# guptakhil/show-tell

Measured on AMD Instinct MI355X. Metric: training images/sec (ResNet101+GRU, emb=512, bs=128) at 1/2/4/8 MI355X, higher is better.
Workload: dtype bf16; 1 GPU; BASELINE configs[1]: ResNet-101 (train-mode BN, frozen) + 5-layer GRU decoder, E=H=512, V=10000, fwd+bwd+SGD step, synthetic COCO-shaped batch; batch_per_gpu=128, global_batch=128, image=3x224x224, parallelism=dp1

## Files before the change

### include/showtell_hip.h

```cpp
#ifndef SHOWTELL_HIP_H
#define SHOWTELL_HIP_H

#include <stddef.h>
#include <stdint.h>

#ifdef __cplusplus
extern "C" {
#endif

#define ST_F32 0
#define ST_BF16 1

#define ST_CELL_GRU 0
#define ST_CELL_LSTM 1

const char* st_last_error(void);
int st_version(void);

typedef struct {
  const void* x;
  const void* w;
  void* y;
  const float* bias;
  const float* scale;
// ... 51 lines not shown
#endif
typedef struct {
  const void* raw2; const void* w3_frag; const void* identity; void* x_out; const void* w1_frag; void* y;
  float* stats; int stats_replicas;
  const float* bn2_stats; const float* bn2_gamma; const float* bn2_beta; int bn2_replicas;
  const float* bn3_stats; const float* bn3_gamma; const float* bn3_beta; int bn3_replicas;
  const float* id_stats; const float* id_gamma; const float* id_beta; int id_replicas;
  float count; float eps;
  long rows; int C1, C2, N;
} st_conv_b2b_desc;
int st_conv_b2b_supported(int C1, int C2, int N);
int st_conv_b2b(const st_conv_b2b_desc* d, void* stream);
typedef struct {
  const void* x2; const void* w3_frag; const void* identity; void* x_out; const void* w1_frag; void* y;
  float* stats; int stats_replicas;
  const float* bn2_stats; const float* bn2_gamma; const float* bn2_beta; int bn2_replicas;
  const float* bn3_stats; const float* bn3_gamma; const float* bn3_beta; int bn3_replicas;
  float count; float eps;
  const float* scale3; const float* shift3; const float* scale1; const float* shift1; int relu1;
  long rows; int C1, C2, N;
  const float* id_stats; const float* id_gamma; const float* id_beta; int id_replicas;
} st_conv_c3c1_desc;
int st_conv_c3c1_supported(int C1, int C2, int N);
int st_conv_c3c1(const st_conv_c3c1_desc* d, void* stream);
int st_conv1x1_astat_supported(int C, int N);
int st_conv1x1_astat(const st_conv1x1_wreg_desc* d, void* stream);

int st_pack_conv_weight_frag(const float* w, void* out, int Cout, int Cin, int KH, int KW, int ntw, void* stream);

int st_tune(int reserved, int kc, int w8);
int st_prof_enable(int on);
int st_debug_stamps(unsigned long long* buf);
int st_prof_collect(double* ms, double* flops, long* launches);

typedef struct {
  const void* x; void* y; const void* res;
  const float* stats;  const float* gamma; const float* beta;
  const float* running_mean; const float* running_var;
  const float* res_stats; const float* res_gamma; const float* res_beta;
  const float* res_running_mean; const float* res_running_var;
  int res_bn;
  int dtype; long rows; int C; float count; float eps; int relu;
  int stats_replicas, res_stats_replicas;
} st_bn_act_desc;

int st_bn_act(const st_bn_act_desc* d, void* stream);

int st_bn_update_running(const float* stats, float* running_mean, float* running_var,
                         int C, float count, float momentum, void* stream);

int st_nchw_to_nhwc(const float* x, void* y, int dtype, int B, int C, int H, int W, int Cpad, void* stream);
int st_nchw_to_s2d16(const float* x, void* y, int dtype, int B, int H, int W, void* stream);
int st_stem_weight_s2d(const void* w, void* out, int dtype, int Cpad, void* stream);
int st_nhwc_to_ncp_f32(const void* x, float* y, int dtype, int B, int HW, int C, void* stream);
int st_maxpool3x3s2(const void* x, void* y, int dtype, int B, int H, int W, int C, void* stream);
int st_maxpool3x3s2_bn(const void* x, void* y, int dtype, int B, int H, int W, int C,
                       const float* stats, const float* gamma, const float* beta,
                       const float* running_mean, const float* running_var, float count, float eps, void* stream);
typedef struct {
  const void* x_s2d; const void* w_frag; void* y;
  float* stats; int stats_replicas;
  const float* gamma;
  const float* scale; const float* shift;
  int B, H, W;
} st_stem_conv_pool_desc;
int st_stem_conv_pool(const st_stem_conv_pool_desc* d, void* stream);
// ... 174 lines not shown
```

### show-tell_amd/_lib.py

```python
import ctypes as C
import os

_HERE = os.path.dirname(os.path.abspath(__file__))
LIB_PATH = os.path.join(_HERE, "lib", "libshowtell_hip.so")

ST_F32, ST_BF16 = 0, 1
ST_CELL_GRU, ST_CELL_LSTM = 0, 1

c_p, c_i, c_f, c_l = C.c_void_p, C.c_int, C.c_float, C.c_long


class ConvDesc(C.Structure):
    _fields_ = [("x", c_p), ("w", c_p), ("y", c_p), ("bias", c_p), ("scale", c_p), ("shift", c_p),
                ("residual", c_p), ("stats", c_p), ("dtype", c_i), ("out_dtype", c_i),
                ("B", c_i), ("Hin", c_i), ("Win", c_i), ("Cin", c_i), ("Ho", c_i), ("Wo", c_i), ("N", c_i),
                ("KH", c_i), ("KW", c_i), ("stride", c_i), ("pad", c_i),
                ("ldx", c_i), ("ldw", c_i), ("ldy", c_i), ("relu", c_i), ("accumulate", c_i), ("Cin_logical", c_i), ("k_order", c_i), ("stats_replicas", c_i),
                ("in_stats", c_p), ("in_gamma", c_p), ("in_beta", c_p), ("in_count", c_f), ("in_eps", c_f), ("split_k", c_i)]


class Conv3x3ImgDesc(C.Structure):
    _fields_ = [("x", c_p), ("w_frag", c_p), ("y", c_p), ("stats", c_p), ("stats_replicas", c_i), ("scale", c_p), ("shift", c_p),
                ("relu", c_i), ("in_stats", c_p), ("in_gamma", c_p), ("in_beta", c_p), ("in_count", c_f), ("in_eps", c_f),
                ("B", c_i), ("H", c_i), ("W", c_i), ("C", c_i), ("N", c_i), ("in_stats_replicas", c_i)]
# ... 75 lines not shown
                ("rows_b", c_p), ("rows_t", c_p), ("prev_row", c_p), ("caption", c_p)]


class ImageBatchDesc(C.Structure):
    _fields_ = [("src", c_p), ("src_bytes", C.c_int64), ("offset", c_p), ("height", c_p), ("width", c_p), ("flip", c_p), ("batch", c_i),
                ("max_height", c_i), ("max_width", c_i), ("out_h", c_i), ("out_w", c_i), ("lut", c_p), ("tmp", c_p),
                ("out", c_p), ("out_u8", c_p)]


_SIGS = {
    "st_version": ([], c_i),
    "st_image_transform": ([C.POINTER(ImageBatchDesc), c_p], c_i),
    "st_conv": ([C.POINTER(ConvDesc), c_p], c_i),
    "st_conv_batch": ([C.POINTER(ConvDesc), c_i, c_p], c_i),
    "st_conv3x3_img_supported": ([c_i, c_i, c_i, c_i], c_i),
    "st_conv3x3_img": ([C.POINTER(Conv3x3ImgDesc), c_p], c_i),
    "st_conv3x3_s2_supported": ([c_i, c_i], c_i),
    "st_conv3x3_s2": ([C.POINTER(Conv3x3ImgDesc), c_p], c_i),
    "st_conv1x1_wreg_supported": ([c_i, c_i], c_i),
    "st_conv1x1_wreg": ([C.POINTER(Conv1x1WregDesc), c_p], c_i),
    "st_conv1x1_kfuse": ([C.POINTER(Conv1x1KfuseDesc), c_p], c_i),
    "st_conv1x1_kfuse_supported": ([c_i, c_i], c_i),
    "st_conv1x1_kfuse8": ([C.POINTER(Conv1x1KfuseDesc), c_p], c_i),
    "st_conv_b2b": ([C.POINTER(ConvB2bDesc), c_p], c_i),
    "st_conv_b2b_supported": ([c_i, c_i, c_i], c_i),
    "st_conv1x1_astat_supported": ([c_i, c_i], c_i),
    "st_conv1x1_astat": ([C.POINTER(Conv1x1WregDesc), c_p], c_i),
    "st_conv1x1_kstream_supported": ([c_i, c_i], c_i),
    "st_conv1x1_kstream": ([C.POINTER(Conv1x1WregDesc), c_p], c_i),
    "st_pack_conv_weight_frag": ([c_p, c_p, c_i, c_i, c_i, c_i, c_i, c_p], c_i),
    "st_tune": ([c_i, c_i, c_i], c_i),
    "st_prof_enable": ([c_i], c_i),
    "st_debug_stamps": ([c_p], c_i),
    "st_prof_collect": ([C.POINTER(C.c_double), C.POINTER(C.c_double), C.POINTER(c_l)], c_i),
    "st_bn_act": ([C.POINTER(BnActDesc), c_p], c_i),
    "st_bn_update_running": ([c_p, c_p, c_p, c_i, c_f, c_f, c_p], c_i),
    "st_nchw_to_nhwc": ([c_p, c_p, c_i, c_i, c_i, c_i, c_i, c_i, c_p], c_i),
    "st_nchw_to_s2d16": ([c_p, c_p, c_i, c_i, c_i, c_i, c_p], c_i),
    "st_stem_weight_s2d": ([c_p, c_p, c_i, c_i, c_p], c_i),
    "st_stem_weight_frag": ([c_p, c_p, c_p], c_i),
    "st_stem_weight_frag_packed": ([c_p, c_i, c_p, c_p], c_i),
    "st_stem_conv_pool": ([C.POINTER(StemConvPoolDesc), c_p], c_i),
    "st_nhwc_to_ncp_f32": ([c_p, c_p, c_i, c_i, c_i, c_i, c_p], c_i),
    "st_maxpool3x3s2": ([c_p, c_p, c_i, c_i, c_i, c_i, c_i, c_p], c_i),
    "st_maxpool3x3s2_bn": ([c_p, c_p, c_i, c_i, c_i, c_i, c_i, c_p, c_p, c_p, c_p, c_p, c_f, c_f, c_p], c_i),
    "st_global_avgpool": ([c_p, c_p, c_i, c_i, c_i, c_i, c_i, c_p], c_i),
    "st_cast": ([c_p, c_p, c_i, c_i, c_l, c_p], c_i),
    "st_transpose": ([c_p, c_p, c_i, c_i, c_i, c_i, c_i, c_p], c_i),
    "st_transpose_colsum": ([c_p, c_p, c_p, c_i, c_i, c_i, c_i, c_i, c_p], c_i),
    "st_transpose_batch": ([c_p, c_p, c_p, c_i, c_i, c_i, c_i, c_i, c_i, c_p, c_p, c_p], c_i),
    "st_pack_conv_weight": ([c_p, c_p, c_i, c_i, c_i, c_i, c_i, c_i, c_i, c_p], c_i),
    "st_cast2d": ([c_p, c_p, c_i, c_i, c_i, c_i, c_i, c_i, c_p], c_i),
    "st_rnn_vocab_ld": ([c_i], c_i),
    "st_rnn_workspace_bytes": ([C.POINTER(RnnParams), C.POINTER(PackedSeq)], C.c_size_t),
    "st_rnn_forward": ([C.POINTER(RnnParams), C.POINTER(PackedSeq), c_p, c_p, c_p, C.c_size_t, c_p, c_i, c_i, c_p, c_i, c_p], c_i),
    "st_rnn_fused_loss_supported": ([C.POINTER(RnnParams)], c_i),
    "st_rnn_fused_loss_bytes": ([C.POINTER(RnnParams), C.POINTER(PackedSeq)], C.c_size_t),
    "st_rnn_fused_loss": ([C.POINTER(RnnParams), C.POINTER(PackedSeq), c_p, C.c_size_t, c_p, c_p, C.c_size_t, c_p, c_p], c_i),
    "st_rnn_fused_dlogits": ([C.POINTER(RnnParams), C.POINTER(PackedSeq), c_p, C.c_size_t, c_p, c_p, c_p, c_p, c_i, c_p], c_i),
    "st_rnn_backward": ([C.POINTER(RnnParams), C.POINTER(RnnGrads), C.POINTER(PackedSeq), c_p, c_p, c_i, c_p, c_p, C.c_size_t,
                         c_p, c_p, c_p], c_i),
    "st_rnn_greedy_workspace_bytes": ([C.POINTER(RnnParams), c_i], C.c_size_t),
    "st_rnn_greedy": ([C.POINTER(RnnParams), c_p, c_i, c_i, c_p, C.c_size_t, c_p, c_p, c_p], c_i),
    "st_rnn_greedy_last_route": ([], c_i),
    "st_rnn_step": ([C.POINTER(RnnParams), c_p, c_i, c_p, c_p, c_p, c_p, c_p, c_i, c_p], c_i),
    "st_embedding_rows": ([c_p, c_p, c_p, c_i, c_i, c_i, c_i, c_i, c_p], c_i),
# ... 80 lines not shown
```

### show-tell_amd/csrc/conv_img.hip

```cpp
#include "common.h"
#include "prof.h"
#include <stdlib.h>
#include <stdio.h>

namespace {

struct ImgArgs {
  const bf16_t* x; const bf16_t* w; bf16_t* y;
  float* stats; int srep;
  const float* scale; const float* shift; int relu;
  const float* in_stats; const float* in_gamma; const float* in_beta; float in_count, in_eps; int in_srep;
  int B, H, W, N, Wp, R, bands, nbn;
  unsigned long long* stamps;
};

template <int CTRL> __device__ __forceinline__ float dpp_rot_(float v) {
  return __int_as_float(__builtin_amdgcn_update_dpp(0, __float_as_int(v), CTRL, 0xf, 0xf, true));
}
__device__ __forceinline__ float row16_sum_(float v) {
  v += dpp_rot_<0x128>(v); v += dpp_rot_<0x124>(v); v += dpp_rot_<0x122>(v); v += dpp_rot_<0x121>(v);
  return v;
}
__device__ __forceinline__ f32x4 mfma_bf16(const u32x4& a, const u32x4& b, const f32x4& c) {
  return __builtin_amdgcn_mfma_f32_16x16x32_bf16(*reinterpret_cast<const bf16x8*>(&a), *reinterpret_cast<const bf16x8*>(&b), c, 0, 0, 0);
}

template <int NC, int BNLOC>
__device__ __forceinline__ void block_stats_flush(const float (&es)[NC], const float (&ess)[NC], bool writer, int local, char* smem,
                                                  float* sdst, int chan0, int N, int tid) {
  float* sred = reinterpret_cast<float*>(smem);
  __syncthreads();
  if (writer) {
#pragma unroll
    for (int c = 0; c < NC; ++c) { sred[local + c] = es[c]; sred[BNLOC + local + c] = ess[c]; }
  }
  __syncthreads();
  for (int t = tid; t < 2 * BNLOC; t += 256) atomicAdd(sdst + (t < BNLOC ? chan0 + t : N + chan0 + t - BNLOC), sred[t]);
}

__device__ __forceinline__ void bn_relu_chunk(u32x4& v, const float* sc, const float* sh);

template <int C, int TM, int NTW, int HALVES, bool AFFINE, int MS = 1>
__device__ __forceinline__ void conv3x3_img_body(const ImgArgs& a) {
  constexpr int TMW = TM / MS;
  static_assert(TM % MS == 0 && (MS == 1 || MS == 2) && (MS == 1 || HALVES == 1), "position split");
  constexpr int PIX = 2 * C + 32;
  constexpr int CS = C / 32;
  constexpr int CSH = CS / HALVES;
  constexpr int KS = 9 * CS;
  constexpr int CH8 = C / 8;
  constexpr int PSTEP = 256 / CH8;
  constexpr bool ALLW = KS * NTW * 4 <= 96;
  extern __shared__ __attribute__((aligned(16))) char smem[];

  const int tid = threadIdx.x, lane = tid & 63;
  const int wid = __builtin_amdgcn_readfirstlane(tid >> 6);
  int lid;
  {
    const int nblk = gridDim.x, id = blockIdx.x, xcd = id & 7, q = nblk >> 3, r = nblk & 7;
    lid = (xcd < r ? xcd * (q + 1) : r * (q + 1) + (xcd - r) * q) + (id >> 3);
  }
  const int nb = lid % a.nbn;
  const int bi = lid / a.nbn;
  const int band = bi % a.bands, img = bi / a.bands;
  const int r0 = band * a.R;
  const int rows = a.H - r0 < a.R ? a.H - r0 : a.R;
  const int Wp = a.Wp;

#define IMG_STAMP(i) do { if (a.stamps && lane == 0) a.stamps[((size_t)blockIdx.x * 4 + wid) * 8 + (i)] = __builtin_amdgcn_s_memtime(); } while (0)
  IMG_STAMP(0);
  constexpr int NSH = C > 256 ? C / 256 : 1;
  StatHead shd[NSH];
  if (a.in_stats) {
#pragma unroll
    for (int k = 0; k < NSH; ++k) { const int c = (tid + 256 * k) % C; stat_head_issue(shd[k], a.in_stats, a.in_srep, C, c, a.in_gamma, a.in_beta); }
  }
  const int r16 = lane & 15, q4 = lane >> 4;
  const int wn = MS == 1 ? wid : (wid & 1), wm = MS == 1 ? 0 : (wid >> 1);
  const int T0 = (nb * (4 / MS) + wn) * NTW;
  const u32x4* wl = reinterpret_cast<const u32x4*>(a.w) + lane;
  constexpr int WQ = ALLW ? KS : CS;
  u32x4 wq[WQ][NTW];
#pragma unroll
  for (int s = 0; s < WQ; ++s)
#pragma unroll
    for (int j = 0; j < NTW; ++j) wq[s][j] = wl[((size_t)(T0 + j) * KS + s) * 64];

  constexpr int CHH = CH8 / 2, U2 = TM >= 14 ? 19 : TM + 3;
  u32x4 v1[HALVES == 2 ? U2 : 1]; bool ok1[HALVES == 2 ? U2 : 1];
  float sc1[8], sh1[8];
  const int cch2 = tid % CHH, pp2 = tid / CHH;
  const bool xf_ = a.in_stats != nullptr;
  if constexpr (HALVES == 2) {
    const int total = 16 * TM + 2 * Wp + 2;
    float* coef = reinterpret_cast<float*>(smem + (size_t)total * PIX);
    const bf16_t* ximg = a.x + (size_t)img * a.H * a.W * C + cch2 * 8;
    u32x4 v0[U2];
    int pr = pp2 / Wp, pc = pp2 - pr * Wp;
#pragma unroll
    for (int u = 0; u < U2; ++u) {
      const int hi = r0 - 1 + pr, wi = pc - 1;
      ok1[u] = pr < rows + 2 && (unsigned)hi < (unsigned)a.H && (unsigned)wi < (unsigned)a.W;
      const int hc = hi < 0 ? 0 : (hi >= a.H ? a.H - 1 : hi), wc = wi < 0 ? 0 : (wi >= a.W ? a.W - 1 : wi);
      v0[u] = *reinterpret_cast<const u32x4*>(ximg + (size_t)(hc * a.W + wc) * C);
      v1[u] = *reinterpret_cast<const u32x4*>(ximg + (size_t)(hc * a.W + wc) * C + C / 2);
      if (!ok1[u]) { v0[u] = u32x4{0u, 0u, 0u, 0u}; v1[u] = u32x4{0u, 0u, 0u, 0u}; }
      pc += 16;
      while (pc >= Wp) { pc -= Wp; ++pr; }
    }
    float sc0[8], sh0[8];
    if (xf_) {
      const float inv = 1.0f / a.in_count;
#pragma unroll
      for (int k = 0; k < NSH; ++k) {
        const int c = tid + 256 * k;
        if (c < C) stat_head_finish(shd[k], a.in_stats, a.in_srep, C, c, inv, a.in_eps, coef[c], coef[C + c]);
      }
      __syncthreads();
#pragma unroll
      for (int e = 0; e < 8; ++e) {
        sc0[e] = coef[cch2 * 8 + e]; sh0[e] = coef[C + cch2 * 8 + e];
        sc1[e] = coef[C / 2 + cch2 * 8 + e]; sh1[e] = coef[C + C / 2 + cch2 * 8 + e];
      }
    }
#pragma unroll
    for (int u = 0; u < U2; ++u) {
      if (xf_ && ok1[u]) bn_relu_chunk(v0[u], sc0, sh0);
      if (pp2 + 16 * u < total) *reinterpret_cast<u32x4*>(smem + (size_t)(pp2 + 16 * u) * PIX + cch2 * 16) = v0[u];
    }
  } else
  {
    const int cch = tid % CH8;
    float sc[8], sh[8];
    const bool xf = a.in_stats != nullptr;
    const int total = 16 * TM + 2 * Wp + 2;
    float* coef = reinterpret_cast<float*>(smem + (size_t)total * PIX);
    const bf16_t* ximg = a.x + (size_t)img * a.H * a.W * C + cch * 8;
    int pp = tid / CH8;
    int pr = pp / Wp, pc = pp - pr * Wp;
    constexpr int U = C == 256 ? 33 : C == 128 ? 18 : C == 64 ? 12 : 21;
    bool first = true;
    for (; pp < total; pp += U * PSTEP) {
      u32x4 v[U]; bool ok[U]; int dst[U];
#pragma unroll
      for (int u = 0; u < U; ++u) {
        const int hi = r0 - 1 + pr, wi = pc - 1;
        ok[u] = pr < rows + 2 && (unsigned)hi < (unsigned)a.H && (unsigned)wi < (unsigned)a.W;
        dst[u] = pp + u * PSTEP < total ? (pp + u * PSTEP) * PIX + cch * 16 : -1;
        const int hc = hi < 0 ? 0 : (hi >= a.H ? a.H - 1 : hi), wc = wi < 0 ? 0 : (wi >= a.W ? a.W - 1 : wi);
        v[u] = *reinterpret_cast<const u32x4*>(ximg + (size_t)(hc * a.W + wc) * C);
        if (!ok[u]) v[u] = u32x4{0u, 0u, 0u, 0u};
        pc += PSTEP;
        while (pc >= Wp) { pc -= Wp; ++pr; }
      }
      if (xf && first) {
        const float inv = 1.0f / a.in_count;
#pragma unroll
        for (int k = 0; k < NSH; ++k) {
          const int c = tid + 256 * k;
          if (c < C) stat_head_finish(shd[k], a.in_stats, a.in_srep, C, c, inv, a.in_eps, coef[c], coef[C + c]);
        }
        __syncthreads();
#pragma unroll
        for (int e = 0; e < 8; ++e) { sc[e] = coef[cch * 8 + e]; sh[e] = coef[C + cch * 8 + e]; }
        first = false;
      }
#pragma unroll
      for (int u = 0; u < U; ++u) {
        if (xf && ok[u]) {
#pragma unroll
          for (int d = 0; d < 4; ++d) {
            const float lo = fmaxf(__uint_as_float(v[u][d] << 16) * sc[2 * d] + sh[2 * d], 0.f);
            const float hi = fmaxf(__uint_as_float(v[u][d] & 0xffff0000u) * sc[2 * d + 1] + sh[2 * d + 1], 0.f);
            v[u][d] = pack_bf16x2(lo, hi);
          }
        }
        if (dst[u] >= 0) *reinterpret_cast<u32x4*>(smem + dst[u]) = v[u];
      }
    }
  }
  IMG_STAMP(1);
  __syncthreads();
  IMG_STAMP(2);

  f32x4 acc[TMW][NTW];
#pragma unroll
  for (int i = 0; i < TMW; ++i)
#pragma unroll
    for (int j = 0; j < NTW; ++j) acc[i][j] = f32x4{0.f, 0.f, 0.f, 0.f};

  constexpr int TH = TMW > 7 ? 7 : TMW;
  const char* abase = smem + (wm * TMW * 16 + r16) * PIX + q4 * 16;
  auto read_a = [&](u32x4 (&fa)[TMW], int s) {
    const int half = s / (9 * CSH), tap = (s / CSH) % 9, cs = half * CSH + s % CSH;
    const char* ab = abase + ((tap / 3) * Wp + tap % 3) * PIX;
    const char* ab2 = ab + TH * 16 * PIX;
#pragma unroll
    for (int i = 0; i < TMW; ++i)
      fa[i] = i < TH ? *reinterpret_cast<const u32x4*>(ab + i * 16 * PIX + cs * 64) : *reinterpret_cast<const u32x4*>(ab2 + (i - TH) * 16 * PIX + cs * 64);
  };
  u32x4 fa0[TMW], fa1[TMW];
  read_a(fa0, 0);
#pragma clang loop unroll(full)
  for (int s = 0; s < KS; ++s) {
    u32x4 (&cur)[TMW] = (s & 1) ? fa1 : fa0;
    u32x4 (&nxt)[TMW] = (s & 1) ? fa0 : fa1;
    constexpr int SPLIT = HALVES == 2 ? KS / 2 : -1;
    if (s + 1 < KS && s + 1 != SPLIT) read_a(nxt, s + 1);
#pragma unroll
    for (int i = 0; i < TMW; ++i)
#pragma unroll
      for (int j = 0; j < NTW; ++j) acc[i][j] = mfma_bf16(wq[s % WQ][j], cur[i], acc[i][j]);
    if (s + WQ < KS) {
#pragma unroll
      for (int j = 0; j < NTW; ++j) wq[s % WQ][j] = wl[((size_t)(T0 + j) * KS + s + WQ) * 64];
    }
    if constexpr (HALVES == 2) {
      if (s < U2) {
        if (xf_ && ok1[s]) bn_relu_chunk(v1[s], sc1, sh1);
        if (pp2 + 16 * s < 16 * TM + 2 * Wp + 2) *reinterpret_cast<u32x4*>(smem + (size_t)(pp2 + 16 * s) * PIX + C + cch2 * 16) = v1[s];
      }
    }
    __builtin_amdgcn_sched_barrier(0);
    if constexpr (HALVES == 2) {
      if (s + 1 == SPLIT) { __syncthreads(); read_a(nxt, s + 1); }
    }
  }

  IMG_STAMP(3);
  constexpr int NC = 4 * NTW;
  const int cb = T0 * 16 + NC * q4;
  float es[NC], ess[NC], scv[NC], shv[NC];
#pragma unroll
  for (int c = 0; c < NC; ++c) { es[c] = 0.f; ess[c] = 0.f; scv[c] = 1.f; shv[c] = 0.f; }
  if constexpr (AFFINE) {
#pragma unroll
    for (int c = 0; c < NC; ++c) { scv[c] = a.scale[cb + c]; shv[c] = a.shift[cb + c]; }
#pragma unroll
    for (int c = 0; c < NC; ++c) asm volatile("" : "+v"(scv[c]), "+v"(shv[c]));
  }
  int ho = r0, wo = r16 + wm * TMW * 16;
  while (wo >= Wp) { wo -= Wp; ++ho; }
  const long yimg = ((long)img * a.H * a.W * a.N + cb) * 2;
#pragma unroll
  for (int i = 0; i < TMW; ++i) {
    const bool valid = wo < a.W && ho < r0 + rows;
    if (valid) {
      float v[NC];
#pragma unroll
      for (int j = 0; j < NTW; ++j)
#pragma unroll
        for (int e = 0; e < 4; ++e) v[4 * j + e] = acc[i][j][e];
#pragma unroll
      for (int c = 0; c < NC; ++c) { es[c] += v[c]; ess[c] += v[c] * v[c]; }
      if constexpr (AFFINE) {
#pragma unroll
        for (int c = 0; c < NC; ++c) v[c] = v[c] * scv[c] + shv[c];
        if (a.relu) {
// ... 17 lines not shown
  if (a.stats) {
    float* sdst = a.stats + (a.srep > 1 ? (size_t)(bi % a.srep) * 2 * a.N : 0);
#pragma unroll
    for (int c = 0; c < NC; ++c) { es[c] = row16_sum_(es[c]); ess[c] = row16_sum_(ess[c]); }
    if constexpr (MS == 1) {
      block_stats_flush<NC, 64 * NTW>(es, ess, r16 == 0, wid * 16 * NTW + NC * q4, smem, sdst, nb * 64 * NTW, a.N, tid);
    } else {
      constexpr int BNLOC = (4 / MS) * 16 * NTW;
      float* sred = reinterpret_cast<float*>(smem);
      const int local = wn * 16 * NTW + NC * q4;
      __syncthreads();
      if (r16 == 0 && wm == 0) {
#pragma unroll
        for (int c = 0; c < NC; ++c) { sred[local + c] = es[c]; sred[BNLOC + local + c] = ess[c]; }
      }
      __syncthreads();
      if (r16 == 0 && wm == 1) {
#pragma unroll
        for (int c = 0; c < NC; ++c) { sred[local + c] += es[c]; sred[BNLOC + local + c] += ess[c]; }
      }
      __syncthreads();
      const int chan0 = nb * BNLOC;
      for (int t = tid; t < 2 * BNLOC; t += 256) atomicAdd(sdst + (t < BNLOC ? chan0 + t : a.N + chan0 + t - BNLOC), sred[t]);
    }
  }
  IMG_STAMP(4);
#undef IMG_STAMP
}

template <int C, int TM, int NTW, int HALVES, bool AFFINE>
__global__ __launch_bounds__(256) __attribute__((amdgpu_waves_per_eu(1, 1))) void conv3x3_img_kernel(ImgArgs a) {
  conv3x3_img_body<C, TM, NTW, HALVES, AFFINE>(a);
}
template <int C, int TM, int NTW, int HALVES, bool AFFINE>
__global__ __launch_bounds__(256, 2) void conv3x3_img_kernel_occ2(ImgArgs a) {
  conv3x3_img_body<C, TM, NTW, HALVES, AFFINE, (C == 64 ? 2 : 1)>(a);
}

struct PwArgs {
  const bf16_t* x; const bf16_t* w; bf16_t* y;
  float* stats; int srep;
  const float* scale; const float* shift; int relu;
  const float* in_stats; const float* in_gamma; const float* in_beta; float in_count, in_eps; int in_srep;
  int M, N, nbn, nstage, spb, mbs;
  int Hin, Win, Ho, Wo, stride;
  const bf16_t* res; bf16_t* xout;
  const float* res_stats; const float* res_gamma; const float* res_beta; int res_srep;
  const bf16_t* idn;
};

__device__ __forceinline__ void bn_relu_chunk(u32x4& v, const float* sc, const float* sh) {
#pragma unroll
  for (int d = 0; d < 4; ++d) {
    const float lo = fmaxf(__uint_as_float(v[d] << 16) * sc[2 * d] + sh[2 * d], 0.f);
    const float hi = fmaxf(__uint_as_float(v[d] & 0xffff0000u) * sc[2 * d + 1] + sh[2 * d + 1], 0.f);
    v[d] = pack_bf16x2(lo, hi);
  }
}

template <int K, int NTW, int TMS, int D, bool STRIDED, bool AFFINE, bool FUSE = false, bool RES = false>
__global__ __launch_bounds__(256) void conv1x1_wreg_kernel(PwArgs a) {
  static_assert(!RES || (AFFINE && !STRIDED && !FUSE), "the residual epilogue is the eval-mode conv3 form");
  constexpr int PIX = 2 * K + 32;
  constexpr int KS = K / 32;
  constexpr int CH8 = K / 8;
  constexpr int SM = 16 * TMS;
  constexpr int RPP = 256 / CH8;
  constexpr int NL = SM / RPP;
  static_assert(SM % RPP == 0 && NL >= 1, "stage/loader mismatch");
// ... 923 lines not shown
}

#endif

__global__ void pack_frag_kernel(const float* __restrict__ w, bf16_t* __restrict__ out, int Cout, int Cin, int KH, int KW, int ntw, int halves) {
  const long total = (long)Cout * KH * KW * Cin;
  const int KS = KH * KW * Cin / 32;
  const int CH = Cin / halves;
  for (long idx = (long)blockIdx.x * blockDim.x + threadIdx.x; idx < total; idx += (long)gridDim.x * blockDim.x) {
    const int j = idx & 7, lane = (idx >> 3) & 63;
    const long f = idx >> 9;
    const int ks = (int)(f % KS), T = (int)(f / KS);
    const int r16 = lane & 15, q4 = lane >> 4;
    const int ch = (T / ntw) * 16 * ntw + 4 * ntw * (r16 >> 2) + 4 * (T % ntw) + (r16 & 3);
    const int kk = 32 * ks + 8 * q4 + j;
    const int half = kk / (KH * KW * CH), rem = kk - half * KH * KW * CH;
    const int tap = rem / CH, c = half * CH + rem - tap * CH;
    const int kh = tap / KW, kw = tap - kh * KW;
    out[idx] = (bf16_t)w[(((long)ch * Cin + c) * KH + kh) * KW + kw];
  }
}

struct ImgCfg { int tm, ntw; };
inline bool img_cfg(int C, int N, ImgCfg* c) {
  switch (C) {
    case 64:  *c = ImgCfg{16, 2}; return N % 64 == 0;
    case 128: *c = ImgCfg{14, 2}; return N % 128 == 0;
    case 256: *c = ImgCfg{14, 2}; return N % 128 == 0;
    case 512: *c = ImgCfg{4, 2};  return N % 128 == 0;
  }
  return false;
}

template <int C, int TM, int NTW, int HALVES, bool AFFINE>
int launch_img_(const ImgArgs& a, int lds, hipStream_t st, double flops) {
  static int attr_set[64] = {};
  int dev = 0;
  (void)hipGetDevice(&dev);
  constexpr bool OCC2 = C == 64 || (C == 256 && TM == 7);
  if (dev >= 0 && dev < 64 && attr_set[dev] < lds) {
    if constexpr (OCC2) (void)hipFuncSetAttribute(reinterpret_cast<const void*>(&conv3x3_img_kernel_occ2<C, TM, NTW, HALVES, AFFINE>), hipFuncAttributeMaxDynamicSharedMemorySize, 160 * 1024);
    else (void)hipFuncSetAttribute(reinterpret_cast<const void*>(&conv3x3_img_kernel<C, TM, NTW, HALVES, AFFINE>), hipFuncAttributeMaxDynamicSharedMemorySize, 160 * 1024);
    attr_set[dev] = 160 * 1024;
  }
  StProfScope prof(C == 64 ? 8 : C == 128 ? 9 : C == 256 ? 10 : 11, flops, st);
  if constexpr (OCC2) hipLaunchKernelGGL((conv3x3_img_kernel_occ2<C, TM, NTW, HALVES, AFFINE>), dim3(a.B * a.bands * a.nbn), dim3(256), lds, st, a);
  else hipLaunchKernelGGL((conv3x3_img_kernel<C, TM, NTW, HALVES, AFFINE>), dim3(a.B * a.bands * a.nbn), dim3(256), lds, st, a);
  prof.end(st);
  ST_LAUNCH_CHECK();
  return 0;
}

template <int C, int TM, int NTW, int HALVES>
int launch_img(const ImgArgs& a, int lds, hipStream_t st, double flops) {
  return a.scale ? launch_img_<C, TM, NTW, HALVES, true>(a, lds, st, flops) : launch_img_<C, TM, NTW, HALVES, false>(a, lds, st, flops);
}
}

extern "C" int st_conv3x3_img_supported(int H, int W, int C, int N) {
  ImgCfg c;
  if (!img_cfg(C, N, &c)) return 0;
  const int Wp = W + 2;
  if (H < 1 || W < 1 || 16 * c.tm < Wp) return 0;
  const long lds = (long)(16 * c.tm + 2 * Wp + 2) * (2 * C + 32) + 2 * C * (long)sizeof(float);
  return lds <= 160 * 1024 ? (c.ntw | (C == 256 ? 2 << 8 : 0)) : 0;
}

extern "C" int st_conv3x3_img(const st_conv3x3_img_desc* d, void* stream) {
  ST_CHECK(d && d->x && d->w_frag && d->y, "st_conv3x3_img: null pointer");
  ImgCfg c;
  ST_CHECK(st_conv3x3_img_supported(d->H, d->W, d->C, d->N) > 0 && img_cfg(d->C, d->N, &c),
           "st_conv3x3_img: unsupported geometry H=%d W=%d C=%d N=%d", d->H, d->W, d->C, d->N);
  ST_CHECK(d->B > 0 && (long)d->B * d->H * d->W * (d->C > d->N ? d->C : d->N) < (1L << 31), "st_conv3x3_img: bad batch");
  ST_CHECK((d->scale == nullptr) == (d->shift == nullptr) && (d->scale || !d->relu), "st_conv3x3_img: scale, shift (and relu) go together");
  ST_CHECK(!d->in_stats || (d->in_gamma && d->in_beta && d->in_count > 0.f), "st_conv3x3_img: input transform needs gamma, beta, count");
  ST_CHECK(d->stats_replicas >= 0 && d->stats_replicas <= 1024 && d->in_stats_replicas >= 0 && d->in_stats_replicas <= 1024, "st_conv3x3_img: bad stats_replicas");
  ImgArgs a;
  a.x = reinterpret_cast<const bf16_t*>(d->x); a.w = reinterpret_cast<const bf16_t*>(d->w_frag); a.y = reinterpret_cast<bf16_t*>(d->y);
  a.stats = d->stats; a.srep = d->stats_replicas; a.scale = d->scale; a.shift = d->shift; a.relu = d->relu;
  a.in_stats = d->in_stats; a.in_gamma = d->in_gamma; a.in_beta = d->in_beta; a.in_count = d->in_count; a.in_eps = d->in_eps; a.in_srep = d->in_stats_replicas > 1 ? d->in_stats_replicas : 1;
  a.B = d->B; a.H = d->H; a.W = d->W; a.N = d->N; a.Wp = d->W + 2;
  static const bool half_env = [] { const char* e = getenv("ST_IMG256_HALF"); return !e || atoi(e) != 0; }();
  const bool half256 = half_env && d->C == 256 && d->W + 2 <= 16 && d->H > 7 * 16 / (d->W + 2);
  if (half256) c.tm = 7;
  a.R = 16 * c.tm / a.Wp; if (a.R > d->H) a.R = d->H;
  a.bands = (d->H + a.R - 1) / a.R;
  a.nbn = d->C == 64 ? d->N / (32 * c.ntw) : d->N / (64 * c.ntw);
  a.stamps = st_debug_stamps_ptr();
  const int lds = (16 * c.tm + 2 * a.Wp + 2) * (2 * d->C + 32) + 2 * d->C * (int)sizeof(float);
  hipStream_t st = reinterpret_cast<hipStream_t>(stream);
  const double flops = 2.0 * d->B * d->H * d->W * (double)d->N * 9.0 * d->C;
  switch (d->C) {
    case 64:  return launch_img<64, 16, 2, 1>(a, lds, st, flops);
    case 128: return launch_img<128, 14, 2, 1>(a, lds, st, flops);
    case 256: return half256 ? launch_img<256, 7, 2, 2>(a, lds, st, flops) : launch_img<256, 14, 2, 2>(a, lds, st, flops);
    case 512: return launch_img<512, 4, 2, 1>(a, lds, st, flops);
  }
  st_set_error("st_conv3x3_img: no kernel for C=%d", d->C);
  return 1;
}

namespace {
struct PwCfg { int ntw, tms; };
inline bool pw_cfg(int K, int N, PwCfg* c) {
  static const int force = [] { const char* e = getenv("ST_PW_CFG"); int a = 0, b = 0; if (e && sscanf(e, "%d,%d", &a, &b) == 2) return a * 100 + b; return 0; }();
  if (N % 64 || (K != 64 && K != 128 && K != 256 && K != 512)) return false;
  if (force) {
    const int ntw = force / 100, tms = force % 100;
    const bool ok = N % (64 * ntw) == 0 && ((ntw == 1 && (tms == 2 || tms == 4)) || (ntw == 2 && (tms == 2 || tms == 4)) || (ntw == 4 && tms == 4));
    if (ok) { *c = PwCfg{ntw, tms}; return true; }
  }
  const bool n128 = N % 128 == 0;
  switch (K) {
    case 64:  *c = N == 64 ? PwCfg{1, 4} : PwCfg{2, 4}; return N == 64 || n128;
    case 128: *c = n128 ? PwCfg{2, 2} : PwCfg{1, 2}; return true;
    case 256: *c = n128 ? PwCfg{2, 4} : PwCfg{1, 2}; return true;
    case 512: *c = n128 ? PwCfg{2, 2} : PwCfg{1, 2}; return true;
  }
  return false;
}

template <int K, int NTW, int TMS, int D, bool STRIDED, bool AFFINE, bool FUSE = false, bool RES = false>
int launch_pw___(PwArgs& a, hipStream_t st, double flops, bool xf) {
  constexpr int SM = 16 * TMS, PIX = 2 * K + 32;
  const int lds = 2 * SM * PIX + (xf ? (FUSE ? 4 : 2) * K * (int)sizeof(float) : 0);
  a.nbn = a.N / (64 * NTW);
  a.nstage = (a.M + SM - 1) / SM;
  static int attr_set[64] = {};
  static int occ_dev[64] = {};
// ... 304 lines not shown
```

### show-tell_amd/csrc/conv_s2.hip

```cpp
#include "common.h"
#include "prof.h"

namespace {

struct S2Args {
  const bf16_t* x; const bf16_t* w; bf16_t* y;
  float* stats; int srep;
  const float* scale; const float* shift; int relu;
  const float* in_stats; const float* in_gamma; const float* in_beta; float in_count, in_eps; int in_srep;
  int M, N, nbn, Hin, Win, Ho, Wo;
};

template <int CTRL> __device__ __forceinline__ float dpp_rot_(float v) {
  return __int_as_float(__builtin_amdgcn_update_dpp(0, __float_as_int(v), CTRL, 0xf, 0xf, true));
}
__device__ __forceinline__ float row16_sum_(float v) {
  v += dpp_rot_<0x128>(v); v += dpp_rot_<0x124>(v); v += dpp_rot_<0x122>(v); v += dpp_rot_<0x121>(v);
  return v;
}
__device__ __forceinline__ f32x4 mfma_bf16(const u32x4& a, const u32x4& b, const f32x4& c) {
  return __builtin_amdgcn_mfma_f32_16x16x32_bf16(*reinterpret_cast<const bf16x8*>(&a), *reinterpret_cast<const bf16x8*>(&b), c, 0, 0, 0);
}

template <int C, int NTW, bool XF, bool AFFINE>
__global__ __launch_bounds__(256) __attribute__((amdgpu_waves_per_eu(C <= 256 ? 2 : 1, C <= 256 ? 2 : 1))) void conv3x3s2_kstream_kernel(S2Args a) {
  constexpr int TM = 7, BM = 16 * TM;
  constexpr int SLAB = 128, PIX = 2 * SLAB + 32, KSS = SLAB / 32;
  constexpr int SPT = C / SLAB;
  constexpr int NSLAB = 9 * SPT, KS = 9 * C / 32;
  constexpr int SLAB_BYTES = BM * PIX;
  constexpr int NL = BM * (SLAB / 8) / 256;
  constexpr int WR = NTW == 4 ? 6 : (C <= 256 ? 4 : 8);
  extern __shared__ __attribute__((aligned(16))) char smem[];
  float* coef = reinterpret_cast<float*>(smem + 2 * SLAB_BYTES);

  const int tid = threadIdx.x, lane = tid & 63;
  const int wid = __builtin_amdgcn_readfirstlane(tid >> 6);
  int lid;
  {
    const int nblk = gridDim.x, id = blockIdx.x, xcd = id & 7, q = nblk >> 3, r = nblk & 7;
    lid = (xcd < r ? xcd * (q + 1) : r * (q + 1) + (xcd - r) * q) + (id >> 3);
  }
  const int nb = lid % a.nbn, bm = lid / a.nbn;
  const int r16 = lane & 15, q4 = lane >> 4;

  constexpr int NSH = C > 256 ? C / 256 : 1;
  StatHead shd[NSH];
  if constexpr (XF) {
#pragma unroll
    for (int k = 0; k < NSH; ++k) { const int c = (tid + 256 * k) % C; stat_head_issue(shd[k], a.in_stats, a.in_srep, C, c, a.in_gamma, a.in_beta); }
  }

  const __amdgpu_buffer_rsrc_t rs_w = __builtin_amdgcn_make_buffer_rsrc(const_cast<bf16_t*>(a.w), 0, 0x7fffffff, 0x00020000);
  const int voffw = (((nb * 4 + wid) * NTW) * KS * 64 + lane) * 16;
  auto wfrag = [&](int ks, int j) { return __builtin_amdgcn_raw_buffer_load_b128(rs_w, voffw, (j * KS + ks) * 1024, 0); };

  const int cch = tid & 15, lrow = tid >> 4;
  int pix0[NL]; unsigned tmask[NL];
#pragma unroll
  for (int i = 0; i < NL; ++i) {
    int m = bm * BM + lrow + 16 * i;
    m = m < a.M ? m : a.M - 1;
    const int hw = a.Ho * a.Wo, b = m / hw, rem = m - b * hw, ho = rem / a.Wo, wo = rem - ho * a.Wo;
    pix0[i] = (b * a.Hin + 2 * ho) * a.Win + 2 * wo;
    unsigned mk = 0;
// ... 131 lines not shown
        if (a.relu) {
#pragma unroll
          for (int c = 0; c < NC; ++c) v[c] = fmaxf(v[c], 0.f);
        }
      }
      const long dst = ((long)m * a.N + cb) * 2;
      if constexpr (NTW == 1) st_out_store8(a.y, dst, u32x2{pack_bf16x2(v[0], v[1]), pack_bf16x2(v[2], v[3])});
      else {
#pragma unroll
        for (int h = 0; h < NTW / 2; ++h)
          st_out_store16(a.y, dst + 16 * h, u32x4{pack_bf16x2(v[8 * h], v[8 * h + 1]), pack_bf16x2(v[8 * h + 2], v[8 * h + 3]),
                                                  pack_bf16x2(v[8 * h + 4], v[8 * h + 5]), pack_bf16x2(v[8 * h + 6], v[8 * h + 7])});
      }
    }
  }
  if (a.stats) {
    float* sdst = a.stats + (a.srep > 1 ? (size_t)(bm % a.srep) * 2 * a.N : 0);
#pragma unroll
    for (int c = 0; c < NC; ++c) { es[c] = row16_sum_(es[c]); ess[c] = row16_sum_(ess[c]); }
    constexpr int BNLOC = 64 * NTW;
    float* sred = reinterpret_cast<float*>(smem);
    const int local = wid * 16 * NTW + NC * q4;
    __syncthreads();
    if (r16 == 0) {
#pragma unroll
      for (int c = 0; c < NC; ++c) { sred[local + c] = es[c]; sred[BNLOC + local + c] = ess[c]; }
    }
    __syncthreads();
    const int chan0 = nb * BNLOC;
    for (int t = tid; t < 2 * BNLOC; t += 256) atomicAdd(sdst + (t < BNLOC ? chan0 + t : a.N + chan0 + t - BNLOC), sred[t]);
  }
}

template <int C, int NTW, bool XF, bool AFFINE>
int launch_s2__(S2Args& a, hipStream_t st, double flops) {
  constexpr int lds = 2 * 112 * (2 * 128 + 32) + 2 * C * 4;
  static int attr_set[64] = {};
  int dev = 0;
  (void)hipGetDevice(&dev);
  if (dev >= 0 && dev < 64 && !attr_set[dev]) {
    (void)hipFuncSetAttribute(reinterpret_cast<const void*>(&conv3x3s2_kstream_kernel<C, NTW, XF, AFFINE>), hipFuncAttributeMaxDynamicSharedMemorySize, lds);
    attr_set[dev] = 1;
  }
  a.nbn = a.N / (64 * NTW);
  StProfScope prof(23, flops, st);
  hipLaunchKernelGGL((conv3x3s2_kstream_kernel<C, NTW, XF, AFFINE>), dim3(((a.M + 111) / 112) * a.nbn), dim3(256), lds, st, a);
  prof.end(st);
  ST_LAUNCH_CHECK();
  return 0;
}
template <int C, int NTW>
int launch_s2(S2Args& a, hipStream_t st, double flops) {
  if (a.in_stats) return a.scale ? launch_s2__<C, NTW, true, true>(a, st, flops) : launch_s2__<C, NTW, true, false>(a, st, flops);
  return a.scale ? launch_s2__<C, NTW, false, true>(a, st, flops) : launch_s2__<C, NTW, false, false>(a, st, flops);
}

}

extern "C" int st_conv3x3_s2_supported(int C, int N) {
  if (C == 128 && N == 128) return 2;
  if (C == 256 && N == 256) return 2;
  if (C == 512 && N == 512) return 2;
  return 0;
}

extern "C" int st_conv3x3_s2(const st_conv3x3_img_desc* d, void* stream) {
  ST_CHECK(d && d->x && d->w_frag && d->y, "st_conv3x3_s2: null pointer");
  ST_CHECK(st_conv3x3_s2_supported(d->C, d->N), "st_conv3x3_s2: unsupported geometry C=%d N=%d", d->C, d->N);
  ST_CHECK(d->B > 0 && d->H >= 1 && d->W >= 1 && (long)d->B * d->H * d->W * d->C * 2 < (1L << 31), "st_conv3x3_s2: bad geometry");
  ST_CHECK((d->scale == nullptr) == (d->shift == nullptr) && (d->scale || !d->relu), "st_conv3x3_s2: scale, shift (and relu) go together");
  ST_CHECK(!d->in_stats || (d->in_gamma && d->in_beta && d->in_count > 0.f), "st_conv3x3_s2: input transform needs gamma, beta, count");
  ST_CHECK(d->stats_replicas >= 0 && d->stats_replicas <= 1024 && d->in_stats_replicas >= 0 && d->in_stats_replicas <= 1024, "st_conv3x3_s2: bad stats_replicas");
  S2Args a{};
  a.x = reinterpret_cast<const bf16_t*>(d->x); a.w = reinterpret_cast<const bf16_t*>(d->w_frag); a.y = reinterpret_cast<bf16_t*>(d->y);
  a.stats = d->stats; a.srep = d->stats_replicas; a.scale = d->scale; a.shift = d->shift; a.relu = d->relu;
  a.in_stats = d->in_stats; a.in_gamma = d->in_gamma; a.in_beta = d->in_beta; a.in_count = d->in_count; a.in_eps = d->in_eps;
  a.in_srep = d->in_stats_replicas > 1 ? d->in_stats_replicas : 1;
  a.Hin = d->H; a.Win = d->W; a.Ho = (d->H - 1) / 2 + 1; a.Wo = (d->W - 1) / 2 + 1;
  a.M = d->B * a.Ho * a.Wo; a.N = d->N;
  hipStream_t st = reinterpret_cast<hipStream_t>(stream);
  const double flops = 2.0 * (double)a.M * d->N * 9.0 * d->C;
  if (d->C == 128) return launch_s2<128, 2>(a, st, flops);
  if (d->C == 256) return launch_s2<256, 2>(a, st, flops);
  return launch_s2<512, 2>(a, st, flops);
}
```

### show-tell_amd/csrc/prof.h

```cpp
#pragma once
#include <hip/hip_runtime.h>

constexpr int kProfVariants = 32;
struct StProfScope {
  bool on = false; size_t idx = 0;
  StProfScope(int variant, double flops, hipStream_t st);
  void end(hipStream_t st);
};

unsigned long long* st_debug_stamps_ptr();
```

### show-tell_amd/csrc/runtime.cpp

```cpp
#include "common.h"
#include <string.h>

static thread_local char g_err[512] = "";

void st_set_error(const char* fmt, ...) {
  va_list ap;
  va_start(ap, fmt);
  vsnprintf(g_err, sizeof(g_err), fmt, ap);
  va_end(ap);
}

extern "C" const char* st_last_error(void) { return g_err; }
extern "C" int st_version(void) { return 1; }
```

Baseline: 31870 images/sec.

## Stage C=512 conv3x3 channel halves sequentially and shrink s2 tile for occupancy 2

For the C=512 stride-1 3x3 conv, the kernel now stages the two input channel halves one after the other into a half-sized LDS buffer, reorders weight prefetch to match, and launches with occupancy 2. For the 512-channel stride-2 conv that has an input transform, it uses a smaller M tile (TM=4) so two blocks fit per CU. Both paths aim to raise latency hiding through more resident waves, at the cost of an extra barrier and restaging, smaller tiles and less weight reuse. Environment switches allow turning each off, and a small query function reports which form ran.

```diff
diff --git a/include/showtell_hip.h b/include/showtell_hip.h
--- a/include/showtell_hip.h
+++ b/include/showtell_hip.h
@@ -107,6 +107,7 @@
 int st_prof_enable(int on);
 int st_debug_stamps(unsigned long long* buf);
 int st_prof_collect(double* ms, double* flops, long* launches);
+int st_conv_last_form(void);
 
 typedef struct {
   const void* x; void* y; const void* res;
diff --git a/show-tell_amd/_lib.py b/show-tell_amd/_lib.py
--- a/show-tell_amd/_lib.py
+++ b/show-tell_amd/_lib.py
@@ -131,6 +131,7 @@
     "st_tune": ([c_i, c_i, c_i], c_i),
     "st_prof_enable": ([c_i], c_i),
     "st_debug_stamps": ([c_p], c_i),
+    "st_conv_last_form": ([], c_i),
     "st_prof_collect": ([C.POINTER(C.c_double), C.POINTER(C.c_double), C.POINTER(c_l)], c_i),
     "st_bn_act": ([C.POINTER(BnActDesc), c_p], c_i),
     "st_bn_update_running": ([c_p, c_p, c_p, c_i, c_f, c_f, c_p], c_i),
diff --git a/show-tell_amd/csrc/conv_img.hip b/show-tell_amd/csrc/conv_img.hip
--- a/show-tell_amd/csrc/conv_img.hip
+++ b/show-tell_amd/csrc/conv_img.hip
@@ -40,11 +40,12 @@
 
 __device__ __forceinline__ void bn_relu_chunk(u32x4& v, const float* sc, const float* sh);
 
-template <int C, int TM, int NTW, int HALVES, bool AFFINE, int MS = 1>
+template <int C, int TM, int NTW, int HALVES, bool AFFINE, int MS = 1, bool SEQ = false>
 __device__ __forceinline__ void conv3x3_img_body(const ImgArgs& a) {
   constexpr int TMW = TM / MS;
   static_assert(TM % MS == 0 && (MS == 1 || MS == 2) && (MS == 1 || HALVES == 1), "position split");
-  constexpr int PIX = 2 * C + 32;
+  static_assert(!SEQ || HALVES == 2, "sequential staging is of two channel halves");
+  constexpr int PIX = (SEQ ? C : 2 * C) + 32;
   constexpr int CS = C / 32;
   constexpr int CSH = CS / HALVES;
   constexpr int KS = 9 * CS;
@@ -79,14 +80,16 @@
   const int wn = MS == 1 ? wid : (wid & 1), wm = MS == 1 ? 0 : (wid >> 1);
   const int T0 = (nb * (4 / MS) + wn) * NTW;
   const u32x4* wl = reinterpret_cast<const u32x4*>(a.w) + lane;
-  constexpr int WQ = ALLW ? KS : CS;
+  constexpr int WQ = ALLW ? KS : (SEQ ? CSH : CS);
+  auto wks = [](int s) { return SEQ ? ((s / CSH) % 9) * CS + (s / (9 * CSH)) * CSH + s % CSH : s; };
   u32x4 wq[WQ][NTW];
 #pragma unroll
   for (int s = 0; s < WQ; ++s)
 #pragma unroll
-    for (int j = 0; j < NTW; ++j) wq[s][j] = wl[((size_t)(T0 + j) * KS + s) * 64];
-
-  constexpr int CHH = CH8 / 2, U2 = TM >= 14 ? 19 : TM + 3;
+    for (int j = 0; j < NTW; ++j) wq[s][j] = wl[((size_t)(T0 + j) * KS + wks(s)) * 64];
+
+  constexpr int CHH = CH8 / 2, PS2 = 256 / CHH;
+  constexpr int U2 = SEQ ? 11 : (TM >= 14 ? 19 : TM + 3);
   u32x4 v1[HALVES == 2 ? U2 : 1]; bool ok1[HALVES == 2 ? U2 : 1];
   float sc1[8], sh1[8];
   const int cch2 = tid % CHH, pp2 = tid / CHH;
@@ -105,7 +108,7 @@
       v0[u] = *reinterpret_cast<const u32x4*>(ximg + (size_t)(hc * a.W + wc) * C);
       v1[u] = *reinterpret_cast<const u32x4*>(ximg + (size_t)(hc * a.W + wc) * C + C / 2);
       if (!ok1[u]) { v0[u] = u32x4{0u, 0u, 0u, 0u}; v1[u] = u32x4{0u, 0u, 0u, 0u}; }
-      pc += 16;
+      pc += PS2;
       while (pc >= Wp) { pc -= Wp; ++pr; }
     }
     float sc0[8], sh0[8];
@@ -126,7 +129,7 @@
 #pragma unroll
     for (int u = 0; u < U2; ++u) {
       if (xf_ && ok1[u]) bn_relu_chunk(v0[u], sc0, sh0);
-      if (pp2 + 16 * u < total) *reinterpret_cast<u32x4*>(smem + (size_t)(pp2 + 16 * u) * PIX + cch2 * 16) = v0[u];
+      if (pp2 + PS2 * u < total) *reinterpret_cast<u32x4*>(smem + (size_t)(pp2 + PS2 * u) * PIX + cch2 * 16) = v0[u];
     }
   } else
   {
@@ -192,7 +195,7 @@
   constexpr int TH = TMW > 7 ? 7 : TMW;
   const char* abase = smem + (wm * TMW * 16 + r16) * PIX + q4 * 16;
   auto read_a = [&](u32x4 (&fa)[TMW], int s) {
-    const int half = s / (9 * CSH), tap = (s / CSH) % 9, cs = half * CSH + s % CSH;
+    const int half = s / (9 * CSH), tap = (s / CSH) % 9, cs = (SEQ ? 0 : half * CSH) + s % CSH;
     const char* ab = abase + ((tap / 3) * Wp + tap % 3) * PIX;
     const char* ab2 = ab + TH * 16 * PIX;
 #pragma unroll
@@ -213,17 +216,28 @@
       for (int j = 0; j < NTW; ++j) acc[i][j] = mfma_bf16(wq[s % WQ][j], cur[i], acc[i][j]);
     if (s + WQ < KS) {
 #pragma unroll
-      for (int j = 0; j < NTW; ++j) wq[s % WQ][j] = wl[((size_t)(T0 + j) * KS + s + WQ) * 64];
-    }
-    if constexpr (HALVES == 2) {
+      for (int j = 0; j < NTW; ++j) wq[s % WQ][j] = wl[((size_t)(T0 + j) * KS + wks(s + WQ)) * 64];
+    }
+    if constexpr (HALVES == 2 && !SEQ) {
       if (s < U2) {
         if (xf_ && ok1[s]) bn_relu_chunk(v1[s], sc1, sh1);
-        if (pp2 + 16 * s < 16 * TM + 2 * Wp + 2) *reinterpret_cast<u32x4*>(smem + (size_t)(pp2 + 16 * s) * PIX + C + cch2 * 16) = v1[s];
+        if (pp2 + PS2 * s < 16 * TM + 2 * Wp + 2) *reinterpret_cast<u32x4*>(smem + (size_t)(pp2 + PS2 * s) * PIX + C + cch2 * 16) = v1[s];
       }
     }
     __builtin_amdgcn_sched_barrier(0);
     if constexpr (HALVES == 2) {
-      if (s + 1 == SPLIT) { __syncthreads(); read_a(nxt, s + 1); }
+      if (s + 1 == SPLIT) {
+        __syncthreads();
+        if constexpr (SEQ) {
+#pragma unroll
+          for (int u = 0; u < U2; ++u) {
+            if (xf_ && ok1[u]) bn_relu_chunk(v1[u], sc1, sh1);
+            if (pp2 + PS2 * u < 16 * TM + 2 * Wp + 2) *reinterpret_cast<u32x4*>(smem + (size_t)(pp2 + PS2 * u) * PIX + cch2 * 16) = v1[u];
+          }
+          __syncthreads();
+        }
+        read_a(nxt, s + 1);
+      }
     }
   }
 
@@ -307,9 +321,9 @@
 __global__ __launch_bounds__(256) __attribute__((amdgpu_waves_per_eu(1, 1))) void conv3x3_img_kernel(ImgArgs a) {
   conv3x3_img_body<C, TM, NTW, HALVES, AFFINE>(a);
 }
-template <int C, int TM, int NTW, int HALVES, bool AFFINE>
+template <int C, int TM, int NTW, int HALVES, bool AFFINE, bool SEQ = false>
 __global__ __launch_bounds__(256, 2) void conv3x3_img_kernel_occ2(ImgArgs a) {
-  conv3x3_img_body<C, TM, NTW, HALVES, AFFINE, (C == 64 ? 2 : 1)>(a);
+  conv3x3_img_body<C, TM, NTW, HALVES, AFFINE, (C == 64 ? 2 : 1), SEQ>(a);
 }
 
 struct PwArgs {
@@ -1299,28 +1313,29 @@
   return false;
 }
 
-template <int C, int TM, int NTW, int HALVES, bool AFFINE>
+template <int C, int TM, int NTW, int HALVES, bool AFFINE, bool SEQ>
 int launch_img_(const ImgArgs& a, int lds, hipStream_t st, double flops) {
   static int attr_set[64] = {};
   int dev = 0;
   (void)hipGetDevice(&dev);
-  constexpr bool OCC2 = C == 64 || (C == 256 && TM == 7);
+  constexpr bool OCC2 = C == 64 || (C == 256 && TM == 7) || SEQ;
   if (dev >= 0 && dev < 64 && attr_set[dev] < lds) {
-    if constexpr (OCC2) (void)hipFuncSetAttribute(reinterpret_cast<const void*>(&conv3x3_img_kernel_occ2<C, TM, NTW, HALVES, AFFINE>), hipFuncAttributeMaxDynamicSharedMemorySize, 160 * 1024);
+    if constexpr (OCC2) (void)hipFuncSetAttribute(reinterpret_cast<const void*>(&conv3x3_img_kernel_occ2<C, TM, NTW, HALVES, AFFINE, SEQ>), hipFuncAttributeMaxDynamicSharedMemorySize, 160 * 1024);
     else (void)hipFuncSetAttribute(reinterpret_cast<const void*>(&conv3x3_img_kernel<C, TM, NTW, HALVES, AFFINE>), hipFuncAttributeMaxDynamicSharedMemorySize, 160 * 1024);
     attr_set[dev] = 160 * 1024;
   }
   StProfScope prof(C == 64 ? 8 : C == 128 ? 9 : C == 256 ? 10 : 11, flops, st);
-  if constexpr (OCC2) hipLaunchKernelGGL((conv3x3_img_kernel_occ2<C, TM, NTW, HALVES, AFFINE>), dim3(a.B * a.bands * a.nbn), dim3(256), lds, st, a);
+  if constexpr (OCC2) hipLaunchKernelGGL((conv3x3_img_kernel_occ2<C, TM, NTW, HALVES, AFFINE, SEQ>), dim3(a.B * a.bands * a.nbn), dim3(256), lds, st, a);
   else hipLaunchKernelGGL((conv3x3_img_kernel<C, TM, NTW, HALVES, AFFINE>), dim3(a.B * a.bands * a.nbn), dim3(256), lds, st, a);
   prof.end(st);
   ST_LAUNCH_CHECK();
   return 0;
 }
 
-template <int C, int TM, int NTW, int HALVES>
+template <int C, int TM, int NTW, int HALVES, bool SEQ = false>
 int launch_img(const ImgArgs& a, int lds, hipStream_t st, double flops) {
-  return a.scale ? launch_img_<C, TM, NTW, HALVES, true>(a, lds, st, flops) : launch_img_<C, TM, NTW, HALVES, false>(a, lds, st, flops);
+  st_note_conv_form(SEQ ? 2 : 1);
+  return a.scale ? launch_img_<C, TM, NTW, HALVES, true, SEQ>(a, lds, st, flops) : launch_img_<C, TM, NTW, HALVES, false, SEQ>(a, lds, st, flops);
 }
 }
 
@@ -1354,14 +1369,16 @@
   a.bands = (d->H + a.R - 1) / a.R;
   a.nbn = d->C == 64 ? d->N / (32 * c.ntw) : d->N / (64 * c.ntw);
   a.stamps = st_debug_stamps_ptr();
-  const int lds = (16 * c.tm + 2 * a.Wp + 2) * (2 * d->C + 32) + 2 * d->C * (int)sizeof(float);
+  const char* seq_env = getenv("ST_IMG512_HALVES");
+  const bool seq512 = !(seq_env && atoi(seq_env) == 0) && d->C == 512 && 16 * c.tm + 2 * a.Wp + 2 <= 88;
+  const int lds = (16 * c.tm + 2 * a.Wp + 2) * ((seq512 ? d->C : 2 * d->C) + 32) + 2 * d->C * (int)sizeof(float);
   hipStream_t st = reinterpret_cast<hipStream_t>(stream);
   const double flops = 2.0 * d->B * d->H * d->W * (double)d->N * 9.0 * d->C;
   switch (d->C) {
     case 64:  return launch_img<64, 16, 2, 1>(a, lds, st, flops);
     case 128: return launch_img<128, 14, 2, 1>(a, lds, st, flops);
     case 256: return half256 ? launch_img<256, 7, 2, 2>(a, lds, st, flops) : launch_img<256, 14, 2, 2>(a, lds, st, flops);
-    case 512: return launch_img<512, 4, 2, 1>(a, lds, st, flops);
+    case 512: return seq512 ? launch_img<512, 4, 2, 2, true>(a, lds, st, flops) : launch_img<512, 4, 2, 1>(a, lds, st, flops);
   }
   st_set_error("st_conv3x3_img: no kernel for C=%d", d->C);
   return 1;
diff --git a/show-tell_amd/csrc/conv_s2.hip b/show-tell_amd/csrc/conv_s2.hip
--- a/show-tell_amd/csrc/conv_s2.hip
+++ b/show-tell_amd/csrc/conv_s2.hip
@@ -1,5 +1,6 @@
 #include "common.h"
 #include "prof.h"
+#include <stdlib.h>
 
 namespace {
 
@@ -22,15 +23,16 @@
   return __builtin_amdgcn_mfma_f32_16x16x32_bf16(*reinterpret_cast<const bf16x8*>(&a), *reinterpret_cast<const bf16x8*>(&b), c, 0, 0, 0);
 }
 
-template <int C, int NTW, bool XF, bool AFFINE>
-__global__ __launch_bounds__(256) __attribute__((amdgpu_waves_per_eu(C <= 256 ? 2 : 1, C <= 256 ? 2 : 1))) void conv3x3s2_kstream_kernel(S2Args a) {
-  constexpr int TM = 7, BM = 16 * TM;
+template <int C, int NTW, bool XF, bool AFFINE, int TM = 7>
+__global__ __launch_bounds__(256) __attribute__((amdgpu_waves_per_eu((C <= 256 || TM < 7) ? 2 : 1, (C <= 256 || TM < 7) ? 2 : 1))) void conv3x3s2_kstream_kernel(S2Args a) {
+  constexpr int BM = 16 * TM;
+  constexpr bool OCC2 = C <= 256 || TM < 7;
   constexpr int SLAB = 128, PIX = 2 * SLAB + 32, KSS = SLAB / 32;
   constexpr int SPT = C / SLAB;
   constexpr int NSLAB = 9 * SPT, KS = 9 * C / 32;
   constexpr int SLAB_BYTES = BM * PIX;
   constexpr int NL = BM * (SLAB / 8) / 256;
-  constexpr int WR = NTW == 4 ? 6 : (C <= 256 ? 4 : 8);
+  constexpr int WR = NTW == 4 ? 6 : (OCC2 ? 4 : 8);
   extern __shared__ __attribute__((aligned(16))) char smem[];
   float* coef = reinterpret_cast<float*>(smem + 2 * SLAB_BYTES);
 
@@ -228,27 +230,28 @@
   }
 }
 
-template <int C, int NTW, bool XF, bool AFFINE>
+template <int C, int NTW, bool XF, bool AFFINE, int TM>
 int launch_s2__(S2Args& a, hipStream_t st, double flops) {
-  constexpr int lds = 2 * 112 * (2 * 128 + 32) + 2 * C * 4;
+  constexpr int BM = 16 * TM, lds = 2 * BM * (2 * 128 + 32) + 2 * C * 4;
   static int attr_set[64] = {};
   int dev = 0;
   (void)hipGetDevice(&dev);
   if (dev >= 0 && dev < 64 && !attr_set[dev]) {
-    (void)hipFuncSetAttribute(reinterpret_cast<const void*>(&conv3x3s2_kstream_kernel<C, NTW, XF, AFFINE>), hipFuncAttributeMaxDynamicSharedMemorySize, lds);
+    (void)hipFuncSetAttribute(reinterpret_cast<const void*>(&conv3x3s2_kstream_kernel<C, NTW, XF, AFFINE, TM>), hipFuncAttributeMaxDynamicSharedMemorySize, lds);
     attr_set[dev] = 1;
   }
   a.nbn = a.N / (64 * NTW);
   StProfScope prof(23, flops, st);
-  hipLaunchKernelGGL((conv3x3s2_kstream_kernel<C, NTW, XF, AFFINE>), dim3(((a.M + 111) / 112) * a.nbn), dim3(256), lds, st, a);
+  hipLaunchKernelGGL((conv3x3s2_kstream_kernel<C, NTW, XF, AFFINE, TM>), dim3(((a.M + BM - 1) / BM) * a.nbn), dim3(256), lds, st, a);
   prof.end(st);
   ST_LAUNCH_CHECK();
   return 0;
 }
-template <int C, int NTW>
+template <int C, int NTW, int TM = 7>
 int launch_s2(S2Args& a, hipStream_t st, double flops) {
-  if (a.in_stats) return a.scale ? launch_s2__<C, NTW, true, true>(a, st, flops) : launch_s2__<C, NTW, true, false>(a, st, flops);
-  return a.scale ? launch_s2__<C, NTW, false, true>(a, st, flops) : launch_s2__<C, NTW, false, false>(a, st, flops);
+  st_note_conv_form((C <= 256 || TM < 7) ? 2 : 1);
+  if (a.in_stats) return a.scale ? launch_s2__<C, NTW, true, true, TM>(a, st, flops) : launch_s2__<C, NTW, true, false, TM>(a, st, flops);
+  return a.scale ? launch_s2__<C, NTW, false, true, TM>(a, st, flops) : launch_s2__<C, NTW, false, false, TM>(a, st, flops);
 }
 
 }
@@ -278,5 +281,10 @@
   const double flops = 2.0 * (double)a.M * d->N * 9.0 * d->C;
   if (d->C == 128) return launch_s2<128, 2>(a, st, flops);
   if (d->C == 256) return launch_s2<256, 2>(a, st, flops);
-  return launch_s2<512, 2>(a, st, flops);
-}
+  const char* env = getenv("ST_S2_512_OCC2");
+  if (a.in_stats && !(env && atoi(env) == 0)) {
+    st_note_conv_form(2);
+    return a.scale ? launch_s2__<512, 2, true, true, 4>(a, st, flops) : launch_s2__<512, 2, true, false, 4>(a, st, flops);
+  }
+  return launch_s2<512, 2, 7>(a, st, flops);
+}
diff --git a/show-tell_amd/csrc/prof.h b/show-tell_amd/csrc/prof.h
--- a/show-tell_amd/csrc/prof.h
+++ b/show-tell_amd/csrc/prof.h
@@ -9,3 +9,4 @@
 };
 
 unsigned long long* st_debug_stamps_ptr();
+void st_note_conv_form(int form);
diff --git a/show-tell_amd/csrc/runtime.cpp b/show-tell_amd/csrc/runtime.cpp
--- a/show-tell_amd/csrc/runtime.cpp
+++ b/show-tell_amd/csrc/runtime.cpp
@@ -1,5 +1,7 @@
 #include "common.h"
+#include "prof.h"
 #include <string.h>
+#include <atomic>
 
 static thread_local char g_err[512] = "";
 
@@ -12,3 +14,7 @@
 
 extern "C" const char* st_last_error(void) { return g_err; }
 extern "C" int st_version(void) { return 1; }
+
+static std::atomic<int> g_conv_form{0};
+void st_note_conv_form(int form) { g_conv_form.store(form, std::memory_order_relaxed); }
+extern "C" int st_conv_last_form(void) { return g_conv_form.load(std::memory_order_relaxed); }
```

New measurement: 32120 images/sec (median of 6 runs). No clear change (+0.8%).
